# nubomedia/NUBOMEDIA-VCA

Measured on AMD Instinct MI355X. Metric: 1080p frames/sec/node (NuboFaceDetector); achieved HBM GB/s vs peak, higher is better.
Workload: dtype i32 rect sums / f32 products / f64 stage sums (u8 pixels)

## Files before the change

nubomedia-vca_amd/csrc/device_records.h:

```cpp
#pragma once
#include <stdint.h>
#include <stddef.h>

#if defined(__HIPCC__)
#define NVCA_HD __host__ __device__
#else
#define NVCA_HD
#endif

namespace nvca {

struct StageRec {
    int first, count; float thr;
    int flags;
    int thr_i;
    int vote_exp;
    int spec_run;
    int pad1;
};

struct ScaleRec {
    int    winw, winh;
    int    plane_off;
    int    pitch;
// ... 57 lines not shown
static constexpr int kTileLdsBudget = 52 * 1024;
static_assert(kTilesPerCu * kTileLdsBudget <= 160 * 1024 && kTilesPerCu * kTileThreads <= 32 * 64, "tile residency per CU");
static constexpr int kTileMaxCols = 256;
NVCA_HD inline int tile_pitch(int ncol) { return ncol | 1; }
NVCA_HD inline int tile_lds_fixed()
{
    return kTileSlots * 8 + 2 * kTileSlots * 2 + 4 * kTileWin + 128 + kTileSlots * 8;
}
NVCA_HD inline int tile_lds_bytes(int ncol, int nrow, int span_x, int span_y)
{
    return 4 * nrow * tile_pitch(ncol) + 2 * ((span_x + 3) & ~3) + 2 * ((span_y + 3) & ~3) + tile_lds_fixed();
}

static constexpr int kStripMaxWin = 512;
static constexpr int kIntegralBand = 16;

struct PreGeom {
    int sw, sh, sstride, cn;
    int w, h, gpitch;
    int spitch;
    int nbands;
    size_t src_slot, gray_slot, sum_slot, band_slot;
};
struct YuvPlanes {
    int fmt, cstride, vstride, pad;
    long long off_y, off_u, off_v;
};
struct ResizeView {
    int mode, xmax;
    const int *xofs; const short *ialpha; const int *yofs; const short *ibeta;
};
struct PyrLevelDev {
    int szw, szh, gpitch, plane_off;
    long long gray_off;
    ResizeView tab;
};
// ... 144 lines not shown
```

nubomedia-vca_amd/csrc/face_stream.cpp:

```cpp
#include "host_state.h"
#include "host_logic.h"
#include <algorithm>
#include <cstdio>
#include <new>

using namespace nvca;

struct nvca_face_stream {
    nvca_ctx *ctx;
    const nvca_cascade *cascade;
    nvca_face_params p;
    Faces faces;
    int num_frame = 0, num_iter = 0, frames_with_no_detection = 0, num_frames_to_process = 0;
    int pending_events = 0;
    nvca_pixel_layout input{};
    const nvca_pixel_layout *yuv() const { return input.format != NVCA_PIX_BGR ? &input : nullptr; }
};

namespace {
constexpr int kGOP = 4;
constexpr int kMaxNoDetection = 1;
constexpr int kNumFramesToProcess = 10;

struct FrameWork {
// ... 233 lines not shown
                hist_clean = nc;
            }
            ws.ln().hist_clean = 0;
            CascadeJob job; job.r0 = gbase + s0; job.n = nc; job.total = n;
            unsigned long long *z_hits = nullptr, *z_deep = nullptr;
            if (!lbp && (rc = cascade_counters(ctx, gp->det, job, &z_hits, &z_deep))) return rc;
            if (yuv) {
              TimedLaunch t(ctx, NVCA_K_GRAY);
              const bool wide = launch_gray_yuv(ctx->cs(), ws.res[ws.cur_res].srcptrs.as<const uint8_t *>() + gbase + s0, gp->g, yuv_planes(yuv), gp->view(),
                              ws.ln().gray.as<uint8_t>(), ws.ln().hist.as<unsigned>(), nc, frames_yuv_aligned16(frames, idx.data() + s0, nc, *yuv));
              if (ctx->sw.plan_debug) fprintf(stderr, "[nvca plan] %s gray of %d frame(s) %d x %d -> %d x %d: %s\n", yuv_is_422(yuv->format) ? "4:2:2" : "4:2:0", nc, f0.width, f0.height, cols, rows, gray_yuv_kernel_name(yuv->format, wide));
            } else
            { TimedLaunch t(ctx, NVCA_K_GRAY);
              launch_gray(ctx->cs(), ws.res[ws.cur_res].srcptrs.as<const uint8_t *>() + gbase + s0, gp->g, gp->view(),
                          ws.ln().gray.as<uint8_t>(), ws.ln().hist.as<unsigned>(), nc, frames_aligned4(frames, idx.data() + s0, nc)); }
            { TimedLaunch t(ctx, NVCA_K_LUT);
              launch_lut(ctx->cs(), ws.ln().hist.as<unsigned>(), cols * rows, ws.ln().lut.as<uint8_t>(), nc, 1, z_hits, z_deep); }
            job.counters_zeroed = !lbp;
            ws.ln().hist_clean = hist_clean;
            if (lbp) {
                const PyrSource src{ws.ln().gray.as<uint8_t>(), gp->g.gpitch, gp->g.gray_slot, ws.ln().lut.as<uint8_t>()};
                if (!scan->lv.empty()) { if ((rc = lbp_launch_set(ctx, scan, src, cols, rows, nc, job, gthr.data() + s0, tk.band_done))) return rc; }
                else { if ((rc = empty_job(ctx, job))) return rc; NVCA_HIP_CHECK(ctx, hipEventRecord(tk.band_done, ctx->cs())); }
            } else {
            run_integral(ctx, gp->g, ws.ln().lut.as<uint8_t>(), nc);
            if (streams[idx[0]]->cascade->c.has_tilted && (rc = run_tilted(ctx, gp->g, ws.ln().lut.as<uint8_t>(), nc))) return rc;
            if ((rc = cascade_enqueue(ctx, gp->det, gp->g.sum_slot, gp->g.spitch, job, gthr.data() + s0, true, tk.band_done))) return rc;
            }
            band_recorded = true;
            jobs.push_back(job);
        }
        gbase += batch;
    }
    if (!band_recorded) NVCA_HIP_CHECK(ctx, hipEventRecord(tk.band_done, ctx->cs()));
    if (!tk.done) NVCA_HIP_CHECK(ctx, hipEventCreateWithFlags(&tk.done, hipEventDisableTiming));
    NVCA_HIP_CHECK(ctx, hipEventRecord(tk.done, ctx->cs()));
    tk.pending = true;
    gates.armed = false;
    return NVCA_OK;
}
// ... 125 lines not shown
```

nubomedia-vca_amd/csrc/host_state.h:

```cpp
#pragma once
#include "context.h"
#include "plan.h"
#include "fb_search.h"
#include "host_math.h"
#include "pyr_levels.h"
#include "yuv_layout.h"

namespace nvca {

bool alloc_log();
void drain_timer_now(nvca_ctx *ctx);
void drain_timer(nvca_ctx *ctx);

struct ResultBufs {
    DevBuf hits, grp, gthr, staging, srcptrs;
    PinnedBuf h_hits, h_grp, h_gthr, h_srcptrs;
    DevBuf recs; PinnedBuf h_recs;
    std::vector<int> gthr_last;
    void release() { hits.release(); grp.release(); gthr.release(); staging.release(); srcptrs.release(); h_hits.release(); h_grp.release(); h_gthr.release(); h_srcptrs.release(); recs.release(); h_recs.release(); gthr_last.clear(); }
};
struct Lane {
    DevBuf gray, hist, lut, bandsum, bandsq, sum, sqsum, tilted, staging, aux, failbits, vnf, deep;
    int hist_clean = 0;
    void release_all()
    {
        gray.release(); hist.release(); lut.release(); bandsum.release(); bandsq.release(); sum.release();
        sqsum.release(); tilted.release(); staging.release(); aux.release();
        failbits.release(); vnf.release(); deep.release();
    }
};
struct Workspace {
    Lane lanes[kLanes];
    int *cur_lane = nullptr;
    Lane &ln() { return lanes[*cur_lane]; }
    ResultBufs res[3];
    int cur_res = 0;
    void release_all()
    {
        for (Lane &l : lanes) l.release_all();
        for (ResultBufs &r : res) r.release();
    }
// ... 41 lines not shown
    unsigned cap = 0;
    size_t first = 0;
    unsigned long long *d_hits = nullptr, *h_hits = nullptr;
    int *d_grp = nullptr, *h_grp = nullptr;
    LevelRec *d_recs = nullptr, *h_recs = nullptr;
};

struct TableBlob {
    std::vector<unsigned char> bytes;
    size_t add(const void *h, size_t n);
    int upload(nvca_ctx *ctx, DevBuf &blob);
};
void make_geom(PreGeom &g, int sw, int sh, int sstride, int cn, int w, int h);
int ensure_ws(nvca_ctx *ctx, const PreGeom &g, int batch);
int upload_tabs(nvca_ctx *ctx, std::vector<std::unique_ptr<GeomPlan>> &levels, DevBuf &blob);
void run_integral(nvca_ctx *ctx, const PreGeom &g, const uint8_t *lut, int batch, const uint8_t *gray = nullptr, int *sum = nullptr,
                  unsigned long long *sq = nullptr);
int run_tilted(nvca_ctx *ctx, const PreGeom &g, const uint8_t *lut, int batch, const uint8_t *gray = nullptr, int *tilted = nullptr);
int cascade_counters(nvca_ctx *ctx, DetectPlan &dp, const CascadeJob &job, unsigned long long **hits, unsigned long long **deep);
int cascade_enqueue(nvca_ctx *ctx, DetectPlan &dp, size_t sum_slot, int spitch, CascadeJob &job, const int *group_thr, bool want_group,
                    hipEvent_t early_done = nullptr );
int group_prepare(nvca_ctx *ctx, CascadeJob &job, const int *group_thr);
int cascade_fetch(nvca_ctx *ctx, CascadeJob &job);
int cascade_collect(nvca_ctx *ctx, DetectPlan &dp, const CascadeJob &job, std::vector<std::vector<nvca_rect>> &raw,
                    std::vector<char> *grouped, std::vector<std::vector<int>> *scale_of = nullptr,
                    std::vector<std::vector<LevelRec>> *recs = nullptr );
void group_all(std::vector<std::vector<nvca_rect>> &raw, int min_neighbors);
GeomPlan *find_plan(nvca_ctx *ctx, const std::string &key);
GeomPlan *store_plan(nvca_ctx *ctx, const std::string &key, std::unique_ptr<GeomPlan> gp);
int get_face_plan(nvca_ctx *ctx, const nvca_cascade *casc, int W, int H, int stride, int cn, int cols, int rows,
                  double sf, int minw, int minh, int maxw, int maxh, GeomPlan **out, const nvca_pixel_layout *yuv = nullptr);
int get_face_pre_plan(nvca_ctx *ctx, int W, int H, int stride, int cn, int cols, int rows, GeomPlan **out, const nvca_pixel_layout *yuv = nullptr);
// ... 98 lines not shown
```

nubomedia-vca_amd/csrc/kernels_equalize.hip:

```cpp
#include "launch.h"
#include "pre_device.h"

namespace nvca {

__global__ __launch_bounds__(256) void k_lut(unsigned *__restrict__ hist, int total, uint8_t *__restrict__ lut, int rezero,
                                             unsigned long long *__restrict__ zero_a, unsigned long long *__restrict__ zero_b)
{
    __shared__ unsigned wsum[4];
    __shared__ unsigned long long wmask[4];
    __shared__ unsigned hs[256];
    const int tid = threadIdx.x, lane = tid & 63, wave = tid >> 6, slot = blockIdx.x;
    const unsigned h = hist[slot * 256 + tid];
    hs[tid] = h;
    if (rezero) hist[slot * 256 + tid] = 0;
    if (slot == 0 && tid == 0) { if (zero_a) *zero_a = 0; if (zero_b) *zero_b = 0; }
    unsigned incl = h;
    for (int d = 1; d < 64; d <<= 1) { unsigned t = __shfl_up(incl, d); if (lane >= d) incl += t; }
    const unsigned long long m = __ballot(h != 0);
    if (lane == 63) wsum[wave] = incl;
    if (lane == 0) wmask[wave] = m;
    __syncthreads();
    for (int j = 0; j < wave; j++) incl += wsum[j];
    int first = 256;
    for (int j = 3; j >= 0; j--) if (wmask[j]) first = j * 64 + __ffsll((long long)wmask[j]) - 1;
    uint8_t out;
    if (first == 256) out = 0;
    else {
        const unsigned hf = hs[first];
        if (hf == (unsigned)total) out = (uint8_t)first;
        else if (tid <= first) out = 0;
        else {
            const float scale = 255.f / (float)(int)(total - (int)hf);
            const float v = (float)(int)(incl - hf) * scale;
            int iv = (int)rintf(v);
            out = (uint8_t)(iv < 0 ? 0 : (iv > 255 ? 255 : iv));
        }
    }
    lut[slot * 256 + tid] = out;
}

void launch_lut(hipStream_t st, unsigned *hist, int total, uint8_t *lut, int batch, int rezero, unsigned long long *zero_a,
                unsigned long long *zero_b)
{
    NVCA_LAUNCH(k_lut, dim3(batch), dim3(256), 0, st, hist, total, lut, rezero, zero_a, zero_b);
}

__global__ __launch_bounds__(256) void k_hist(const uint8_t *__restrict__ gray, int w, int h, int pitch,
                                              unsigned *__restrict__ hist)
{
    __shared__ unsigned lh[4][256];
    const int tid = threadIdx.x, wave = tid >> 6;
    for (int i = tid; i < 1024; i += 256) (&lh[0][0])[i] = 0;
    __syncthreads();
// ... 53 lines not shown
```

nubomedia-vca_amd/csrc/kernels_integral.hip:

```cpp
#include "launch.h"

namespace nvca {

__global__ __launch_bounds__(256) void k_colsum(const uint8_t *__restrict__ gray, const uint8_t *__restrict__ lut,
                                                int lut_stride, PreGeom g, unsigned *__restrict__ bandsum,
                                                unsigned *__restrict__ bandsq)
{
    __shared__ uint8_t sl[256];
    const int tid = threadIdx.x, band = blockIdx.y, slot = blockIdx.z;
    sl[tid] = lut ? lut[(size_t)slot * lut_stride + tid] : (uint8_t)tid;
    __syncthreads();
    const int x4 = (blockIdx.x * 256 + tid) * 4;
    const int bpitch = (int)(g.band_slot / g.nbands);
    if (x4 >= bpitch) return;
    const int y0 = band * kIntegralBand, y1 = min(g.h, y0 + kIntegralBand);
    unsigned s[4] = {0, 0, 0, 0}, q[4] = {0, 0, 0, 0};
    if (x4 < g.w) {
        const uint8_t *base = gray + (size_t)slot * g.gray_slot + x4;
        for (int y = y0; y < y1; y++) {
            const unsigned px = *(const unsigned *)(base + (size_t)y * g.gpitch);
#pragma unroll
            for (int k = 0; k < 4; k++) {
                const unsigned v = (x4 + k < g.w) ? sl[(px >> (8 * k)) & 255] : 0u;
                s[k] += v; q[k] += v * v;
            }
        }
    }
    const size_t o = (size_t)slot * g.band_slot + (size_t)band * bpitch + x4;
    *(uint4 *)(bandsum + o) = make_uint4(s[0], s[1], s[2], s[3]);
    *(uint4 *)(bandsq + o) = make_uint4(q[0], q[1], q[2], q[3]);
}
void launch_colsum(hipStream_t st, const uint8_t *gray, const uint8_t *lut, int lut_stride, const PreGeom &g,
                   unsigned *bandsum, unsigned *bandsq, int batch)
{
    const int bpitch = (int)(g.band_slot / g.nbands);
    dim3 grid((bpitch / 4 + 255) / 256, g.nbands, batch);
    NVCA_LAUNCH(k_colsum, grid, dim3(256), 0, st, gray, lut, lut_stride, g, bandsum, bandsq);
}

__global__ __launch_bounds__(256) void k_bandscan(PreGeom g, unsigned *__restrict__ bandsum, unsigned *__restrict__ bandsq)
{
    const int bpitch = (int)(g.band_slot / g.nbands);
    const int x = blockIdx.x * 256 + threadIdx.x, slot = blockIdx.y;
    if (x >= bpitch) return;
    unsigned rs = 0, rq = 0;
    size_t o = (size_t)slot * g.band_slot + x;
    for (int b0 = 0; b0 < g.nbands; b0 += 16) {
        unsigned ts[16], tq[16];
#pragma unroll
        for (int k = 0; k < 16; k++) {
            const bool in = b0 + k < g.nbands;
            ts[k] = in ? bandsum[o + (size_t)k * bpitch] : 0u; tq[k] = in ? bandsq[o + (size_t)k * bpitch] : 0u;
        }
#pragma unroll
        for (int k = 0; k < 16; k++)
            if (b0 + k < g.nbands) {
                bandsum[o + (size_t)k * bpitch] = rs; bandsq[o + (size_t)k * bpitch] = rq;
                rs += ts[k]; rq += tq[k];
            }
        o += (size_t)16 * bpitch;
    }
}
void launch_bandscan(hipStream_t st, const PreGeom &g, unsigned *bandsum, unsigned *bandsq, int batch)
{
    const int bpitch = (int)(g.band_slot / g.nbands);
    NVCA_LAUNCH(k_bandscan, dim3((bpitch + 255) / 256, batch), dim3(256), 0, st, g, bandsum, bandsq);
}

__device__ __forceinline__ unsigned wave_incl_scan_u32(unsigned v, int lane)
{
    unsigned x = v;
    x += (unsigned)__builtin_amdgcn_update_dpp(0, (int)v, 0x111, 0xf, 0xf, true);
    x += (unsigned)__builtin_amdgcn_update_dpp(0, (int)v, 0x112, 0xf, 0xf, true);
    x += (unsigned)__builtin_amdgcn_update_dpp(0, (int)v, 0x113, 0xf, 0xf, true);
    x += (unsigned)__builtin_amdgcn_update_dpp(0, (int)x, 0x114, 0xf, 0xe, true);
    x += (unsigned)__builtin_amdgcn_update_dpp(0, (int)x, 0x118, 0xf, 0xc, true);
    const unsigned t0 = (unsigned)__builtin_amdgcn_readlane((int)x, 15), t1 = (unsigned)__builtin_amdgcn_readlane((int)x, 31),
                   t2 = (unsigned)__builtin_amdgcn_readlane((int)x, 47);
    const int row = lane >> 4;
    return x + (row >= 1 ? t0 : 0u) + (row >= 2 ? t1 : 0u) + (row >= 3 ? t2 : 0u);
}

static constexpr int kIntThreads = 512;
static constexpr int kIntWaves = kIntThreads / 64;

__global__ __launch_bounds__(kIntThreads) void k_integral(const uint8_t *__restrict__ gray, const uint8_t *__restrict__ lut,
                                                          int lut_stride, PreGeom g, const unsigned *__restrict__ bandsum,
                                                          const unsigned *__restrict__ bandsq, int *__restrict__ sum,
                                                          unsigned *__restrict__ sq32)
{
    __shared__ uint8_t sl[256];
    __shared__ unsigned wrow_s[kIntegralBand][kIntWaves], wrow_q[kIntegralBand][kIntWaves];
    __shared__ unsigned wb_s[kIntWaves];
    __shared__ unsigned long long wb_q[kIntWaves];
    __shared__ unsigned carry_s[kIntegralBand], carry_q[kIntegralBand];
    __shared__ unsigned cbase_s;
    __shared__ unsigned long long cbase_q;
    const int tid = threadIdx.x, lane = tid & 63, wave = tid >> 6;
    const int band = blockIdx.x, slot = blockIdx.y;
    if (tid < 256) sl[tid] = lut ? lut[(size_t)slot * lut_stride + tid] : (uint8_t)tid;
    if (tid < kIntegralBand) { carry_s[tid] = 0; carry_q[tid] = 0; }
    if (tid == 0) { cbase_s = 0; cbase_q = 0; }
    __syncthreads();
    const int y0 = band * kIntegralBand, y1 = min(g.h, y0 + kIntegralBand);
    const int bpitch = (int)(g.band_slot / g.nbands);
    const uint8_t *gbase = gray + (size_t)slot * g.gray_slot;
    int *sbase = sum + (size_t)slot * g.sum_slot;
    unsigned *lbase = sq32 + (size_t)slot * 2 * g.sum_slot;
    uint8_t *hbase = (uint8_t *)(lbase + g.sum_slot);
    const unsigned *bs = bandsum + (size_t)slot * g.band_slot + (size_t)band * bpitch;
    const unsigned *bq = bandsq + (size_t)slot * g.band_slot + (size_t)band * bpitch;
    const int nchunks = (g.w + 1 + 2047) / 2048;

    for (int c = 0; c < nchunks; c++) {
        const int X0 = c * 2048 + tid * 4;
        const bool in_pitch = X0 < g.spitch;
        unsigned ps[4]; unsigned long long pq[4];
        {
            uint4 a = make_uint4(0, 0, 0, 0), e = make_uint4(0, 0, 0, 0);
            if (X0 + 4 <= bpitch) { a = *(const uint4 *)(bs + X0); e = *(const uint4 *)(bq + X0); }
            const unsigned vs[4] = {a.x, a.y, a.z, a.w}, vq[4] = {e.x, e.y, e.z, e.w};
            unsigned rs = 0; unsigned long long rq = 0;
#pragma unroll
            for (int k = 0; k < 4; k++) {
                const bool ok = X0 + k < g.w;
                rs += ok ? vs[k] : 0u; rq += ok ? vq[k] : 0u;
                ps[k] = rs; pq[k] = rq;
            }
        }
        const unsigned ts = ps[3]; const unsigned long long tq = pq[3];
        unsigned is = wave_incl_scan_u32(ts + (tid == 0 ? cbase_s : 0u), lane);
        unsigned long long iq = tq + (tid == 0 ? cbase_q : 0ull);
        for (int d = 1; d < 64; d <<= 1) { const unsigned long long b = __shfl_up(iq, d); if (lane >= d) iq += b; }
        if (lane == 63) { wb_s[wave] = is; wb_q[wave] = iq; }
        __syncthreads();
        for (int j = 0; j < wave; j++) { is += wb_s[j]; iq += wb_q[j]; }
// ... 53 lines not shown
                *(unsigned *)(hbase + o) = (unsigned)(acc_q[0] >> 32) | ((unsigned)(acc_q[1] >> 32) << 8) | ((unsigned)(acc_q[2] >> 32) << 16) |
                                           ((unsigned)(acc_q[3] >> 32) << 24);
            }
            }
        }
        __syncthreads();
        if (tid < kIntegralBand) {
            unsigned ts_ = 0, tq_ = 0;
            for (int j = 0; j < kIntWaves; j++) { ts_ += wrow_s[tid][j]; tq_ += wrow_q[tid][j]; }
            carry_s[tid] += ts_; carry_q[tid] += tq_;
        }
        __syncthreads();
    }
}
void launch_integral(hipStream_t st, const uint8_t *gray, const uint8_t *lut, int lut_stride, const PreGeom &g,
                     const unsigned *bandsum, const unsigned *bandsq, int *sum, unsigned long long *sqsum,
                     int batch)
{
    NVCA_LAUNCH(k_integral, dim3(g.nbands, batch), dim3(kIntThreads), 0, st, gray, lut, lut_stride, g, bandsum,
                       bandsq, sum, (unsigned *)sqsum);
}

static constexpr int kSmallIntWords = 16 * 1024 - 256;
__device__ __forceinline__ void small_integral(const uint8_t *__restrict__ g, int gpitch, const uint8_t *__restrict__ lut, int w, int h,
                                               int *__restrict__ s, unsigned *__restrict__ lo, uint8_t *__restrict__ hi, int P, unsigned *sm)
{
    const int tid = threadIdx.x, lane = tid & 63, wave = tid >> 6, nthreads = blockDim.x, nwaves = nthreads >> 6;
    const int pitch = w | 1;
    for (int X = tid; X <= w; X += nthreads) { s[X] = 0; lo[X] = 0; hi[X] = 0; }
    for (int pass = 0; pass < 2; pass++) {
        for (int y = wave; y < h; y += nwaves) {
            const uint8_t *row = g + (size_t)y * gpitch;
            unsigned carry = 0;
            for (int x0 = 0; x0 < w; x0 += 64) {
                const int x = x0 + lane;
// ... 148 lines not shown
```

nubomedia-vca_amd/csrc/launch.h:

```cpp
#pragma once
#include <hip/hip_runtime.h>
#include <hip/hip_ext.h>
#include "device_records.h"
#include "trk_layout.h"
#include "pixel_rules.h"

namespace nvca {

bool launch_events(hipEvent_t *a, hipEvent_t *b);
void note_launch(const char *kernel);
hipError_t take_launch_error(const char **kernel);
#define NVCA_LAUNCH(kern, grid, block, shmem, st, ...)                                                            \
    do {                                                                                                          \
        hipEvent_t ea__, eb__;                                                                                    \
        if (nvca::launch_events(&ea__, &eb__)) hipExtLaunchKernelGGL(kern, grid, block, shmem, st, ea__, eb__, 0, __VA_ARGS__); \
        else hipLaunchKernelGGL(kern, grid, block, shmem, st, __VA_ARGS__);                                       \
        nvca::note_launch(#kern);                                                                                 \
    } while (0)

void launch_gray(hipStream_t st, const uint8_t *const *d_src, const PreGeom &g, const ResizeView &t,
                 uint8_t *gray, unsigned *hist, int batch, bool aligned4);
bool launch_gray_yuv(hipStream_t st, const uint8_t *const *d_src, const PreGeom &g, const YuvPlanes &p, const ResizeView &t,
                     uint8_t *gray, unsigned *hist, int batch, bool aligned16);
const char *gray_yuv_kernel_name(int fmt, bool wide);
// ... 7 lines not shown
void launch_resize1(hipStream_t st, const uint8_t *src, int sw, int sh, int sstride, const ResizeView &t,
                    uint8_t *dst, int dw, int dh, int dstride, unsigned *hist, int batch = 1, size_t src_slot = 0, size_t dst_slot = 0,
                    const uint8_t *luts = nullptr );
void launch_resize3(hipStream_t st, const uint8_t *src, int sw, int sh, int sstride, const ResizeView &t,
                    uint8_t *dst, int dw, int dh, int dstride);
void launch_flip_h(hipStream_t st, const uint8_t *src, int w, int h, int spitch, uint8_t *dst, int dpitch, int batch = 1, size_t src_slot = 0,
                   size_t dst_slot = 0);
void launch_hist(hipStream_t st, const uint8_t *gray, int w, int h, int pitch, unsigned *hist);
void launch_lut(hipStream_t st, unsigned *hist, int total, uint8_t *lut, int batch, int rezero = 0,
                unsigned long long *zero_a = nullptr, unsigned long long *zero_b = nullptr);
void launch_apply_lut(hipStream_t st, const uint8_t *src, int w, int h, int spitch, const uint8_t *lut,
                      uint8_t *dst, int dpitch, int batch = 1, size_t src_slot = 0, size_t dst_slot = 0);
void launch_work_resize(hipStream_t st, bool bgr, const uint8_t *const *d_srcs, const int *d_lut_idx, const uint8_t *d_luts, int sh, int sstride,
                        const ResizeView &t, uint8_t *dst, int dw, int dh, int dstride, size_t dst_slot, unsigned *hist, int batch, const YuvPlanes *yuv = nullptr);
void launch_colsum(hipStream_t st, const uint8_t *gray, const uint8_t *lut, int lut_stride, const PreGeom &g,
                   unsigned *bandsum, unsigned *bandsq, int batch);
void launch_bandscan(hipStream_t st, const PreGeom &g, unsigned *bandsum, unsigned *bandsq, int batch);
void launch_integral(hipStream_t st, const uint8_t *gray, const uint8_t *lut, int lut_stride, const PreGeom &g,
                     const unsigned *bandsum, const unsigned *bandsq, int *sum, unsigned long long *sqsum,
                     int batch);

bool small_integral_fits(const PreGeom &g);
void launch_small_integral(hipStream_t st, const uint8_t *gray, const uint8_t *lut, int lut_stride, const PreGeom &g, int *sum,
                           unsigned long long *sqsum, int batch);

struct TrkLaunch {
    const TrkSlot *slots; int batch, w, h;
    int fmt;
    bool wide;
    int *labels; CompAcc *acc;
    int *out; int cap;
    uint8_t *flags; int *roots; int roots_cap; int *tiles; int tick;
    int order;
    int rows, rows_uf;
};
// ... 55 lines not shown
```

nubomedia-vca_amd/csrc/plans.cpp:

```cpp
#include "host_state.h"
#include "host_logic.h"
#include <cstdio>
#include <cstring>
#include <algorithm>

using namespace nvca;

namespace nvca {

static RowCopy make_rowcopy(const ResizeTab &t)
{
    RowCopy rc;
    if (t.mode != 1 || t.dh <= 0) return rc;
    std::vector<int> rows;
    auto clampr = [&](int r) { return r >= 0 ? (r < t.sh ? r : t.sh - 1) : 0; };
    for (int dy = 0; dy < t.dh; dy++) { rows.push_back(clampr(t.yofs[dy])); rows.push_back(clampr(t.yofs[dy] + 1)); }
    std::sort(rows.begin(), rows.end());
    rows.erase(std::unique(rows.begin(), rows.end()), rows.end());
    if (rows.size() * 2 > (size_t)t.sh) return rc;
    std::vector<std::pair<int, int>> runs;
    for (int r : rows) { if (!runs.empty() && runs.back().first + runs.back().second == r) runs.back().second++; else runs.push_back({r, 1}); }
    const int period = runs.size() > 1 ? runs[1].first - runs[0].first : t.sh;
    for (size_t i = 0; i < runs.size(); i++)
        if (runs[i].second != runs[0].second || runs[i].first != runs[0].first + (int)i * period) return rc;
// ... 46 lines not shown
    for (auto &it : items) it.d->release();
    int rc;
    if ((rc = blob.upload(ctx, d_blob))) return rc;
    for (auto &it : items) { it.d->p = it.n ? (unsigned char *)d_blob.p + it.off : nullptr; it.d->bytes = 0; }
    return NVCA_OK;
}

void make_geom(PreGeom &g, int sw, int sh, int sstride, int cn, int w, int h)
{
    memset(&g, 0, sizeof(g));
    g.sw = sw; g.sh = sh; g.sstride = sstride; g.cn = cn;
    g.w = w; g.h = h;
    g.gpitch = (int)round_up(w, 64);
    g.spitch = (int)round_up(w + 1, 8);
    g.nbands = (h + kIntegralBand - 1) / kIntegralBand;
    g.gray_slot = round_up((size_t)g.gpitch * h, 256);
    g.sum_slot = round_up((size_t)g.spitch * (h + 1), 64);
    g.band_slot = (size_t)g.nbands * round_up(w, 8);
}

int ensure_ws(nvca_ctx *ctx, const PreGeom &g, int batch)
{
    Workspace &ws = *ctx->ws;
    int e = 0;
    e |= ws.ln().gray.ensure(g.gray_slot * batch + 64);
    { void *old = ws.ln().hist.p; e |= ws.ln().hist.ensure((size_t)batch * 256 * sizeof(unsigned)); if (ws.ln().hist.p != old) ws.ln().hist_clean = 0; }
    e |= ws.ln().lut.ensure((size_t)batch * 256);
    e |= ws.ln().bandsum.ensure(g.band_slot * batch * sizeof(unsigned));
    e |= ws.ln().bandsq.ensure(g.band_slot * batch * sizeof(unsigned));
    e |= ws.ln().sum.ensure((g.sum_slot * batch + 4 * (size_t)g.spitch) * sizeof(int));
    e |= ws.ln().sqsum.ensure(g.sum_slot * batch * sizeof(unsigned long long));
    e |= ws.res[ws.cur_res].srcptrs.ensure((size_t)batch * sizeof(void *));
    e |= ws.res[ws.cur_res].h_srcptrs.ensure((size_t)batch * sizeof(void *));
    if (e) { ctx->set_error("device/pinned allocation failed for the workspace"); return NVCA_ERR_NOMEM; }
    return NVCA_OK;
}

static int upload_tab(nvca_ctx *ctx, GeomPlan &gp)
{
    const ResizeTab &t = gp.tab;
    if (t.mode != 1) return NVCA_OK;
    if (gp.d_xofs.ensure(t.xofs.size() * 4) || gp.d_yofs.ensure(t.yofs.size() * 4) ||
        gp.d_ialpha.ensure(t.ialpha.size() * 2) || gp.d_ibeta.ensure(t.ibeta.size() * 2)) {
        ctx->set_error("hipMalloc failed for resize tables"); return NVCA_ERR_NOMEM;
// ... 14 lines not shown
    std::vector<unsigned char> h(total);
    if (blob.ensure(total)) { ctx->set_error("hipMalloc failed for resize tables"); return NVCA_ERR_NOMEM; }
    size_t off = 0;
    auto put = [&](DevBuf &d, const void *src, size_t n) { memcpy(h.data() + off, src, n); d.release(); d.p = (unsigned char *)blob.p + off; d.bytes = 0; off += al(n); };
    for (auto &gp : levels) {
        const ResizeTab &t = gp->tab;
        if (t.mode != 1) continue;
        put(gp->d_xofs, t.xofs.data(), t.xofs.size() * 4); put(gp->d_yofs, t.yofs.data(), t.yofs.size() * 4);
        put(gp->d_ialpha, t.ialpha.data(), t.ialpha.size() * 2); put(gp->d_ibeta, t.ibeta.data(), t.ibeta.size() * 2);
    }
    NVCA_HIP_CHECK(ctx, hipMemcpy(blob.p, h.data(), total, hipMemcpyHostToDevice));
    return NVCA_OK;
}


void run_integral(nvca_ctx *ctx, const PreGeom &g, const uint8_t *lut, int batch, const uint8_t *gray, int *sum,
                  unsigned long long *sq)
{
    Workspace &ws = *ctx->ws;
    if (!gray) gray = ws.ln().gray.as<uint8_t>();
    if (!sum) sum = ws.ln().sum.as<int>();
    if (!sq) sq = ws.ln().sqsum.as<unsigned long long>();
    if (batch <= 64 && small_integral_fits(g)) {
        TimedLaunch t(ctx, NVCA_K_INTEGRAL);
        launch_small_integral(ctx->cs(), gray, lut, 256, g, sum, sq, batch);
        return;
    }
    { TimedLaunch t(ctx, NVCA_K_COLSUM);
      launch_colsum(ctx->cs(), gray, lut, 256, g, ws.ln().bandsum.as<unsigned>(), ws.ln().bandsq.as<unsigned>(), batch); }
    { TimedLaunch t(ctx, NVCA_K_BANDSCAN);
      launch_bandscan(ctx->cs(), g, ws.ln().bandsum.as<unsigned>(), ws.ln().bandsq.as<unsigned>(), batch); }
    { TimedLaunch t(ctx, NVCA_K_INTEGRAL);
      launch_integral(ctx->cs(), gray, lut, 256, g, ws.ln().bandsum.as<unsigned>(), ws.ln().bandsq.as<unsigned>(), sum, sq, batch); }
}

int run_tilted(nvca_ctx *ctx, const PreGeom &g, const uint8_t *lut, int batch, const uint8_t *gray, int *tilted)
{
    Workspace &ws = *ctx->ws;
    if (g.w + 1 > 8 * 1024 || (size_t)2 * (g.w + g.h + 2) * sizeof(int) > 64 * 1024) { ctx->set_error("image too large for the tilted integral"); return NVCA_ERR_ARG; }
    if (!tilted) {
        if (ws.ln().tilted.ensure((g.sum_slot * batch + 4 * (size_t)g.spitch) * sizeof(int))) { ctx->set_error("device allocation failed (tilted integral)"); return NVCA_ERR_NOMEM; }
        tilted = ws.ln().tilted.as<int>();
    }
    if (!gray) gray = ws.ln().gray.as<uint8_t>();
    TimedLaunch t(ctx, NVCA_K_INTEGRAL);
    launch_tilted(ctx->cs(), gray, lut, 256, g, tilted, batch);
    return NVCA_OK;
}
// ... 305 lines not shown
```

nubomedia-vca_amd/csrc/pre_device.h:

```cpp
#pragma once
#include "launch.h"

#if defined(__HIPCC__)
namespace nvca {

static constexpr int kGrayRows = 8;

__device__ __forceinline__ void hist_flush(unsigned (*lh)[256], unsigned *hist, int tid)
{
    __syncthreads();
    unsigned v = lh[0][tid] + lh[1][tid] + lh[2][tid] + lh[3][tid];
    if (v) atomicAdd(&hist[tid], v);
}

}
#endif
```

Baseline: 21130.

## Fuse histogram-equalize LUT into colsum and scan super-bands instead of all bands

Removes the separate LUT launch on the multi-launch integral path: colsum now builds the equalization LUT from the histogram itself and writes it out once, and bandscan takes over re-zeroing the histogram and counters. Colsum is restructured so each thread loads 16 pixels per row with wide loads across four bands per block and emits band prefixes within a super-band of four bands. The serial band scan then runs only over super-band totals, and the integral kernel adds the super-band prefix back in. This cuts one launch and shortens the serial scan, at the cost of redundant per-block LUT computation and more shared memory and register use in colsum.

```diff
diff --git a/nubomedia-vca_amd/csrc/device_records.h b/nubomedia-vca_amd/csrc/device_records.h
--- a/nubomedia-vca_amd/csrc/device_records.h
+++ b/nubomedia-vca_amd/csrc/device_records.h
@@ -95,12 +95,13 @@
 
 static constexpr int kStripMaxWin = 512;
 static constexpr int kIntegralBand = 16;
+static constexpr int kSuperBands = 4;
 
 struct PreGeom {
     int sw, sh, sstride, cn;
     int w, h, gpitch;
     int spitch;
-    int nbands;
+    int nbands, nsuper;
     size_t src_slot, gray_slot, sum_slot, band_slot;
 };
 struct YuvPlanes {
diff --git a/nubomedia-vca_amd/csrc/face_stream.cpp b/nubomedia-vca_amd/csrc/face_stream.cpp
--- a/nubomedia-vca_amd/csrc/face_stream.cpp
+++ b/nubomedia-vca_amd/csrc/face_stream.cpp
@@ -271,16 +271,20 @@
             { TimedLaunch t(ctx, NVCA_K_GRAY);
               launch_gray(ctx->cs(), ws.res[ws.cur_res].srcptrs.as<const uint8_t *>() + gbase + s0, gp->g, gp->view(),
                           ws.ln().gray.as<uint8_t>(), ws.ln().hist.as<unsigned>(), nc, frames_aligned4(frames, idx.data() + s0, nc)); }
-            { TimedLaunch t(ctx, NVCA_K_LUT);
-              launch_lut(ctx->cs(), ws.ln().hist.as<unsigned>(), cols * rows, ws.ln().lut.as<uint8_t>(), nc, 1, z_hits, z_deep); }
+            const bool chain_lut = !lbp && !integral_in_one_launch(gp->g, nc);
+            const ChainEqualize eq{ws.ln().hist.as<unsigned>(), cols * rows, ws.ln().lut.as<uint8_t>(), z_hits, z_deep};
+            if (!chain_lut) {
+              TimedLaunch t(ctx, NVCA_K_LUT);
+              launch_lut(ctx->cs(), ws.ln().hist.as<unsigned>(), cols * rows, ws.ln().lut.as<uint8_t>(), nc, 1, z_hits, z_deep);
+              ws.ln().hist_clean = hist_clean; }
             job.counters_zeroed = !lbp;
-            ws.ln().hist_clean = hist_clean;
             if (lbp) {
                 const PyrSource src{ws.ln().gray.as<uint8_t>(), gp->g.gpitch, gp->g.gray_slot, ws.ln().lut.as<uint8_t>()};
                 if (!scan->lv.empty()) { if ((rc = lbp_launch_set(ctx, scan, src, cols, rows, nc, job, gthr.data() + s0, tk.band_done))) return rc; }
                 else { if ((rc = empty_job(ctx, job))) return rc; NVCA_HIP_CHECK(ctx, hipEventRecord(tk.band_done, ctx->cs())); }
             } else {
-            run_integral(ctx, gp->g, ws.ln().lut.as<uint8_t>(), nc);
+            run_integral(ctx, gp->g, ws.ln().lut.as<uint8_t>(), nc, nullptr, nullptr, nullptr, chain_lut ? &eq : nullptr);
+            if (chain_lut) ws.ln().hist_clean = hist_clean;
             if (streams[idx[0]]->cascade->c.has_tilted && (rc = run_tilted(ctx, gp->g, ws.ln().lut.as<uint8_t>(), nc))) return rc;
             if ((rc = cascade_enqueue(ctx, gp->det, gp->g.sum_slot, gp->g.spitch, job, gthr.data() + s0, true, tk.band_done))) return rc;
             }
diff --git a/nubomedia-vca_amd/csrc/host_state.h b/nubomedia-vca_amd/csrc/host_state.h
--- a/nubomedia-vca_amd/csrc/host_state.h
+++ b/nubomedia-vca_amd/csrc/host_state.h
@@ -20,11 +20,11 @@
     void release() { hits.release(); grp.release(); gthr.release(); staging.release(); srcptrs.release(); h_hits.release(); h_grp.release(); h_gthr.release(); h_srcptrs.release(); recs.release(); h_recs.release(); gthr_last.clear(); }
 };
 struct Lane {
-    DevBuf gray, hist, lut, bandsum, bandsq, sum, sqsum, tilted, staging, aux, failbits, vnf, deep;
+    DevBuf gray, hist, lut, bandsum, bandsq, supersum, supersq, sum, sqsum, tilted, staging, aux, failbits, vnf, deep;
     int hist_clean = 0;
     void release_all()
     {
-        gray.release(); hist.release(); lut.release(); bandsum.release(); bandsq.release(); sum.release();
+        gray.release(); hist.release(); lut.release(); bandsum.release(); bandsq.release(); supersum.release(); supersq.release(); sum.release();
         sqsum.release(); tilted.release(); staging.release(); aux.release();
         failbits.release(); vnf.release(); deep.release();
     }
@@ -96,8 +96,13 @@
 void make_geom(PreGeom &g, int sw, int sh, int sstride, int cn, int w, int h);
 int ensure_ws(nvca_ctx *ctx, const PreGeom &g, int batch);
 int upload_tabs(nvca_ctx *ctx, std::vector<std::unique_ptr<GeomPlan>> &levels, DevBuf &blob);
+struct ChainEqualize {
+    unsigned *hist; int total; uint8_t *lut;
+    unsigned long long *zero_a, *zero_b;
+};
+bool integral_in_one_launch(const PreGeom &g, int batch);
 void run_integral(nvca_ctx *ctx, const PreGeom &g, const uint8_t *lut, int batch, const uint8_t *gray = nullptr, int *sum = nullptr,
-                  unsigned long long *sq = nullptr);
+                  unsigned long long *sq = nullptr, const ChainEqualize *eq = nullptr );
 int run_tilted(nvca_ctx *ctx, const PreGeom &g, const uint8_t *lut, int batch, const uint8_t *gray = nullptr, int *tilted = nullptr);
 int cascade_counters(nvca_ctx *ctx, DetectPlan &dp, const CascadeJob &job, unsigned long long **hits, unsigned long long **deep);
 int cascade_enqueue(nvca_ctx *ctx, DetectPlan &dp, size_t sum_slot, int spitch, CascadeJob &job, const int *group_thr, bool want_group,
diff --git a/nubomedia-vca_amd/csrc/kernels_equalize.hip b/nubomedia-vca_amd/csrc/kernels_equalize.hip
--- a/nubomedia-vca_amd/csrc/kernels_equalize.hip
+++ b/nubomedia-vca_amd/csrc/kernels_equalize.hip
@@ -6,37 +6,12 @@
 __global__ __launch_bounds__(256) void k_lut(unsigned *__restrict__ hist, int total, uint8_t *__restrict__ lut, int rezero,
                                              unsigned long long *__restrict__ zero_a, unsigned long long *__restrict__ zero_b)
 {
-    __shared__ unsigned wsum[4];
-    __shared__ unsigned long long wmask[4];
-    __shared__ unsigned hs[256];
-    const int tid = threadIdx.x, lane = tid & 63, wave = tid >> 6, slot = blockIdx.x;
+    __shared__ LutScratch sc;
+    const int tid = threadIdx.x, slot = blockIdx.x;
     const unsigned h = hist[slot * 256 + tid];
-    hs[tid] = h;
     if (rezero) hist[slot * 256 + tid] = 0;
     if (slot == 0 && tid == 0) { if (zero_a) *zero_a = 0; if (zero_b) *zero_b = 0; }
-    unsigned incl = h;
-    for (int d = 1; d < 64; d <<= 1) { unsigned t = __shfl_up(incl, d); if (lane >= d) incl += t; }
-    const unsigned long long m = __ballot(h != 0);
-    if (lane == 63) wsum[wave] = incl;
-    if (lane == 0) wmask[wave] = m;
-    __syncthreads();
-    for (int j = 0; j < wave; j++) incl += wsum[j];
-    int first = 256;
-    for (int j = 3; j >= 0; j--) if (wmask[j]) first = j * 64 + __ffsll((long long)wmask[j]) - 1;
-    uint8_t out;
-    if (first == 256) out = 0;
-    else {
-        const unsigned hf = hs[first];
-        if (hf == (unsigned)total) out = (uint8_t)first;
-        else if (tid <= first) out = 0;
-        else {
-            const float scale = 255.f / (float)(int)(total - (int)hf);
-            const float v = (float)(int)(incl - hf) * scale;
-            int iv = (int)rintf(v);
-            out = (uint8_t)(iv < 0 ? 0 : (iv > 255 ? 255 : iv));
-        }
-    }
-    lut[slot * 256 + tid] = out;
+    lut[slot * 256 + tid] = equalize_lut_entry(h, total, tid, sc);
 }
 
 void launch_lut(hipStream_t st, unsigned *hist, int total, uint8_t *lut, int batch, int rezero, unsigned long long *zero_a,
diff --git a/nubomedia-vca_amd/csrc/kernels_integral.hip b/nubomedia-vca_amd/csrc/kernels_integral.hip
--- a/nubomedia-vca_amd/csrc/kernels_integral.hip
+++ b/nubomedia-vca_amd/csrc/kernels_integral.hip
@@ -1,70 +1,152 @@
 #include "launch.h"
+#include "pre_device.h"
 
 namespace nvca {
 
-__global__ __launch_bounds__(256) void k_colsum(const uint8_t *__restrict__ gray, const uint8_t *__restrict__ lut,
-                                                int lut_stride, PreGeom g, unsigned *__restrict__ bandsum,
-                                                unsigned *__restrict__ bandsq)
+static constexpr int kColsumWaves = 4;
+static constexpr int kColsumCols = 64 * 16;
+template <bool kWide>
+__device__ __forceinline__ void colsum_load(uint4 (&px)[kIntegralBand], const uint8_t *__restrict__ p, int pitch, int x0, int w, int nr)
+{
+#pragma unroll
+    for (int r = 0; r < kIntegralBand; r++) {
+        px[r] = make_uint4(0, 0, 0, 0);
+        if (x0 < w && r < nr) {
+            const uint8_t *row = p + (size_t)r * pitch;
+            if (kWide) px[r] = *(const uint4 *)row;
+            else {
+                px[r].x = *(const unsigned *)row;
+                if (x0 + 4 < w) px[r].y = *(const unsigned *)(row + 4);
+                if (x0 + 8 < w) px[r].z = *(const unsigned *)(row + 8);
+                if (x0 + 12 < w) px[r].w = *(const unsigned *)(row + 12);
+            }
+        }
+    }
+}
+template <bool kWide>
+__global__ __launch_bounds__(kColsumWaves * 64) void k_colsum(const uint8_t *__restrict__ gray, const uint8_t *__restrict__ lut, int lut_stride,
+                                                              PreGeom g, unsigned *__restrict__ bandsum, unsigned *__restrict__ bandsq,
+                                                              unsigned *__restrict__ supersum, unsigned *__restrict__ supersq,
+                                                              const unsigned *__restrict__ hist, int total, uint8_t *__restrict__ lut_out)
 {
     __shared__ uint8_t sl[256];
-    const int tid = threadIdx.x, band = blockIdx.y, slot = blockIdx.z;
-    sl[tid] = lut ? lut[(size_t)slot * lut_stride + tid] : (uint8_t)tid;
+    __shared__ LutScratch sc;
+    __shared__ __attribute__((aligned(16))) unsigned sm_s[kSuperBands][kColsumCols], sm_q[kSuperBands][kColsumCols];
+    const int tid = threadIdx.x, lane = tid & 63, wave = __builtin_amdgcn_readfirstlane(tid >> 6);
+    const int sb = blockIdx.y, slot = blockIdx.z;
+    const int bpitch = (int)(g.band_slot / g.nbands);
+    const int xb = blockIdx.x * kColsumCols, x0 = xb + lane * 16;
+    const uint8_t *base = gray + (size_t)slot * g.gray_slot + x0;
+    uint4 px[kIntegralBand];
+    int bi = wave;
+    int y0 = (sb * kSuperBands + bi) * kIntegralBand, nr = min(kIntegralBand, g.h - y0);
+    if (bi < kSuperBands) colsum_load<kWide>(px, base + (size_t)y0 * g.gpitch, g.gpitch, x0, g.w, nr);
+    if (hist) {
+        const uint8_t e = equalize_lut_entry(hist[slot * 256 + tid], total, tid, sc);
+        sl[tid] = e;
+        if (blockIdx.x == 0 && sb == 0) lut_out[(size_t)slot * lut_stride + tid] = e;
+    } else sl[tid] = lut ? lut[(size_t)slot * lut_stride + tid] : (uint8_t)tid;
     __syncthreads();
-    const int x4 = (blockIdx.x * 256 + tid) * 4;
+    while (bi < kSuperBands) {
+        unsigned s[16], q[16];
+#pragma unroll
+        for (int k = 0; k < 16; k++) { s[k] = 0; q[k] = 0; }
+#pragma unroll
+        for (int r = 0; r < kIntegralBand; r++)
+            if (r < nr) {
+                const unsigned wd[4] = {px[r].x, px[r].y, px[r].z, px[r].w};
+#pragma unroll
+                for (int k = 0; k < 16; k++) {
+                    const unsigned v = sl[(wd[k >> 2] >> (8 * (k & 3))) & 255];
+                    s[k] += v; q[k] += v * v;
+                }
+            }
+#pragma unroll
+        for (int k = 0; k < 16; k += 4) {
+            *(uint4 *)&sm_s[bi][lane * 16 + k] = make_uint4(s[k], s[k + 1], s[k + 2], s[k + 3]);
+            *(uint4 *)&sm_q[bi][lane * 16 + k] = make_uint4(q[k], q[k + 1], q[k + 2], q[k + 3]);
+        }
+        bi += kColsumWaves;
+        if (bi < kSuperBands) {
+            y0 = (sb * kSuperBands + bi) * kIntegralBand; nr = min(kIntegralBand, g.h - y0);
+            colsum_load<kWide>(px, base + (size_t)y0 * g.gpitch, g.gpitch, x0, g.w, nr);
+        }
+    }
+    __syncthreads();
+    for (bi = wave; bi < kSuperBands; bi += kColsumWaves) {
+        const int band = sb * kSuperBands + bi;
+        const bool last = bi == kSuperBands - 1;
+        if (band >= g.nbands && !last) continue;
+#pragma unroll
+        for (int i = 0; i < kColsumCols / 256; i++) {
+            const int c = (i * 64 + lane) * 4;
+            if (xb + c + 4 > bpitch) continue;
+            uint4 as = make_uint4(0, 0, 0, 0), aq = make_uint4(0, 0, 0, 0);
+            for (int j = 0; j < bi; j++) {
+                const uint4 ts = *(const uint4 *)&sm_s[j][c], tq = *(const uint4 *)&sm_q[j][c];
+                as.x += ts.x; as.y += ts.y; as.z += ts.z; as.w += ts.w;
+                aq.x += tq.x; aq.y += tq.y; aq.z += tq.z; aq.w += tq.w;
+            }
+            if (band < g.nbands) {
+                const size_t o = (size_t)slot * g.band_slot + (size_t)band * bpitch + xb + c;
+                *(uint4 *)(bandsum + o) = as; *(uint4 *)(bandsq + o) = aq;
+            }
+            if (last) {
+                const uint4 ts = *(const uint4 *)&sm_s[bi][c], tq = *(const uint4 *)&sm_q[bi][c];
+                as.x += ts.x; as.y += ts.y; as.z += ts.z; as.w += ts.w;
+                aq.x += tq.x; aq.y += tq.y; aq.z += tq.z; aq.w += tq.w;
+                const size_t o = ((size_t)slot * g.nsuper + sb) * bpitch + xb + c;
+                *(uint4 *)(supersum + o) = as; *(uint4 *)(supersq + o) = aq;
+            }
+        }
+    }
+}
+void launch_colsum(hipStream_t st, const uint8_t *gray, const uint8_t *lut, int lut_stride, const PreGeom &g,
+                   unsigned *bandsum, unsigned *bandsq, unsigned *supersum, unsigned *supersq, int batch,
+                   const unsigned *hist, int total, uint8_t *lut_out)
+{
     const int bpitch = (int)(g.band_slot / g.nbands);
-    if (x4 >= bpitch) return;
-    const int y0 = band * kIntegralBand, y1 = min(g.h, y0 + kIntegralBand);
-    unsigned s[4] = {0, 0, 0, 0}, q[4] = {0, 0, 0, 0};
-    if (x4 < g.w) {
-        const uint8_t *base = gray + (size_t)slot * g.gray_slot + x4;
-        for (int y = y0; y < y1; y++) {
-            const unsigned px = *(const unsigned *)(base + (size_t)y * g.gpitch);
-#pragma unroll
-            for (int k = 0; k < 4; k++) {
-                const unsigned v = (x4 + k < g.w) ? sl[(px >> (8 * k)) & 255] : 0u;
-                s[k] += v; q[k] += v * v;
-            }
-        }
-    }
-    const size_t o = (size_t)slot * g.band_slot + (size_t)band * bpitch + x4;
-    *(uint4 *)(bandsum + o) = make_uint4(s[0], s[1], s[2], s[3]);
-    *(uint4 *)(bandsq + o) = make_uint4(q[0], q[1], q[2], q[3]);
-}
-void launch_colsum(hipStream_t st, const uint8_t *gray, const uint8_t *lut, int lut_stride, const PreGeom &g,
-                   unsigned *bandsum, unsigned *bandsq, int batch)
-{
-    const int bpitch = (int)(g.band_slot / g.nbands);
-    dim3 grid((bpitch / 4 + 255) / 256, g.nbands, batch);
-    NVCA_LAUNCH(k_colsum, grid, dim3(256), 0, st, gray, lut, lut_stride, g, bandsum, bandsq);
-}
-
-__global__ __launch_bounds__(256) void k_bandscan(PreGeom g, unsigned *__restrict__ bandsum, unsigned *__restrict__ bandsq)
+    dim3 grid((bpitch + kColsumCols - 1) / kColsumCols, g.nsuper, batch);
+    if (!(((uintptr_t)gray | (uintptr_t)g.gpitch | (uintptr_t)g.gray_slot) & 15))
+        NVCA_LAUNCH(k_colsum<true>, grid, dim3(kColsumWaves * 64), 0, st, gray, lut, lut_stride, g, bandsum, bandsq, supersum, supersq, hist, total, lut_out);
+    else
+        NVCA_LAUNCH(k_colsum<false>, grid, dim3(kColsumWaves * 64), 0, st, gray, lut, lut_stride, g, bandsum, bandsq, supersum, supersq, hist, total, lut_out);
+}
+
+__global__ __launch_bounds__(256) void k_bandscan(PreGeom g, unsigned *__restrict__ supersum, unsigned *__restrict__ supersq,
+                                                  unsigned *__restrict__ hist, unsigned long long *__restrict__ zero_a,
+                                                  unsigned long long *__restrict__ zero_b)
 {
     const int bpitch = (int)(g.band_slot / g.nbands);
     const int x = blockIdx.x * 256 + threadIdx.x, slot = blockIdx.y;
+    if (blockIdx.x == 0) {
+        if (hist) hist[slot * 256 + threadIdx.x] = 0;
+        if (slot == 0 && threadIdx.x == 0) { if (zero_a) *zero_a = 0; if (zero_b) *zero_b = 0; }
+    }
     if (x >= bpitch) return;
     unsigned rs = 0, rq = 0;
-    size_t o = (size_t)slot * g.band_slot + x;
-    for (int b0 = 0; b0 < g.nbands; b0 += 16) {
+    size_t o = (size_t)slot * g.nsuper * bpitch + x;
+    for (int b0 = 0; b0 < g.nsuper; b0 += 16) {
         unsigned ts[16], tq[16];
 #pragma unroll
         for (int k = 0; k < 16; k++) {
-            const bool in = b0 + k < g.nbands;
-            ts[k] = in ? bandsum[o + (size_t)k * bpitch] : 0u; tq[k] = in ? bandsq[o + (size_t)k * bpitch] : 0u;
+            const bool in = b0 + k < g.nsuper;
+            ts[k] = in ? supersum[o + (size_t)k * bpitch] : 0u; tq[k] = in ? supersq[o + (size_t)k * bpitch] : 0u;
         }
 #pragma unroll
         for (int k = 0; k < 16; k++)
-            if (b0 + k < g.nbands) {
-                bandsum[o + (size_t)k * bpitch] = rs; bandsq[o + (size_t)k * bpitch] = rq;
+            if (b0 + k < g.nsuper) {
+                supersum[o + (size_t)k * bpitch] = rs; supersq[o + (size_t)k * bpitch] = rq;
                 rs += ts[k]; rq += tq[k];
             }
         o += (size_t)16 * bpitch;
     }
 }
-void launch_bandscan(hipStream_t st, const PreGeom &g, unsigned *bandsum, unsigned *bandsq, int batch)
+void launch_bandscan(hipStream_t st, const PreGeom &g, unsigned *supersum, unsigned *supersq, int batch, unsigned *hist,
+                     unsigned long long *zero_a, unsigned long long *zero_b)
 {
     const int bpitch = (int)(g.band_slot / g.nbands);
-    NVCA_LAUNCH(k_bandscan, dim3((bpitch + 255) / 256, batch), dim3(256), 0, st, g, bandsum, bandsq);
+    NVCA_LAUNCH(k_bandscan, dim3((bpitch + 255) / 256, batch), dim3(256), 0, st, g, supersum, supersq, hist, zero_a, zero_b);
 }
 
 __device__ __forceinline__ unsigned wave_incl_scan_u32(unsigned v, int lane)
@@ -86,7 +168,8 @@
 
 __global__ __launch_bounds__(kIntThreads) void k_integral(const uint8_t *__restrict__ gray, const uint8_t *__restrict__ lut,
                                                           int lut_stride, PreGeom g, const unsigned *__restrict__ bandsum,
-                                                          const unsigned *__restrict__ bandsq, int *__restrict__ sum,
+                                                          const unsigned *__restrict__ bandsq, const unsigned *__restrict__ supersum,
+                                                          const unsigned *__restrict__ supersq, int *__restrict__ sum,
                                                           unsigned *__restrict__ sq32)
 {
     __shared__ uint8_t sl[256];
@@ -110,6 +193,8 @@
     uint8_t *hbase = (uint8_t *)(lbase + g.sum_slot);
     const unsigned *bs = bandsum + (size_t)slot * g.band_slot + (size_t)band * bpitch;
     const unsigned *bq = bandsq + (size_t)slot * g.band_slot + (size_t)band * bpitch;
+    const unsigned *ss = supersum + ((size_t)slot * g.nsuper + band / kSuperBands) * bpitch;
+    const unsigned *sq = supersq + ((size_t)slot * g.nsuper + band / kSuperBands) * bpitch;
     const int nchunks = (g.w + 1 + 2047) / 2048;
 
     for (int c = 0; c < nchunks; c++) {
@@ -118,8 +203,9 @@
         unsigned ps[4]; unsigned long long pq[4];
         {
             uint4 a = make_uint4(0, 0, 0, 0), e = make_uint4(0, 0, 0, 0);
-            if (X0 + 4 <= bpitch) { a = *(const uint4 *)(bs + X0); e = *(const uint4 *)(bq + X0); }
-            const unsigned vs[4] = {a.x, a.y, a.z, a.w}, vq[4] = {e.x, e.y, e.z, e.w};
+            uint4 ta = a, te = e;
+            if (X0 + 4 <= bpitch) { a = *(const uint4 *)(bs + X0); e = *(const uint4 *)(bq + X0); ta = *(const uint4 *)(ss + X0); te = *(const uint4 *)(sq + X0); }
+            const unsigned vs[4] = {a.x + ta.x, a.y + ta.y, a.z + ta.z, a.w + ta.w}, vq[4] = {e.x + te.x, e.y + te.y, e.z + te.z, e.w + te.w};
             unsigned rs = 0; unsigned long long rq = 0;
 #pragma unroll
             for (int k = 0; k < 4; k++) {
@@ -203,11 +289,11 @@
     }
 }
 void launch_integral(hipStream_t st, const uint8_t *gray, const uint8_t *lut, int lut_stride, const PreGeom &g,
-                     const unsigned *bandsum, const unsigned *bandsq, int *sum, unsigned long long *sqsum,
-                     int batch)
+                     const unsigned *bandsum, const unsigned *bandsq, const unsigned *supersum, const unsigned *supersq,
+                     int *sum, unsigned long long *sqsum, int batch)
 {
     NVCA_LAUNCH(k_integral, dim3(g.nbands, batch), dim3(kIntThreads), 0, st, gray, lut, lut_stride, g, bandsum,
-                       bandsq, sum, (unsigned *)sqsum);
+                       bandsq, supersum, supersq, sum, (unsigned *)sqsum);
 }
 
 static constexpr int kSmallIntWords = 16 * 1024 - 256;
diff --git a/nubomedia-vca_amd/csrc/launch.h b/nubomedia-vca_amd/csrc/launch.h
--- a/nubomedia-vca_amd/csrc/launch.h
+++ b/nubomedia-vca_amd/csrc/launch.h
@@ -45,11 +45,13 @@
 void launch_work_resize(hipStream_t st, bool bgr, const uint8_t *const *d_srcs, const int *d_lut_idx, const uint8_t *d_luts, int sh, int sstride,
                         const ResizeView &t, uint8_t *dst, int dw, int dh, int dstride, size_t dst_slot, unsigned *hist, int batch, const YuvPlanes *yuv = nullptr);
 void launch_colsum(hipStream_t st, const uint8_t *gray, const uint8_t *lut, int lut_stride, const PreGeom &g,
-                   unsigned *bandsum, unsigned *bandsq, int batch);
-void launch_bandscan(hipStream_t st, const PreGeom &g, unsigned *bandsum, unsigned *bandsq, int batch);
+                   unsigned *bandsum, unsigned *bandsq, unsigned *supersum, unsigned *supersq, int batch,
+                   const unsigned *hist = nullptr, int total = 0, uint8_t *lut_out = nullptr);
+void launch_bandscan(hipStream_t st, const PreGeom &g, unsigned *supersum, unsigned *supersq, int batch, unsigned *hist = nullptr,
+                     unsigned long long *zero_a = nullptr, unsigned long long *zero_b = nullptr);
 void launch_integral(hipStream_t st, const uint8_t *gray, const uint8_t *lut, int lut_stride, const PreGeom &g,
-                     const unsigned *bandsum, const unsigned *bandsq, int *sum, unsigned long long *sqsum,
-                     int batch);
+                     const unsigned *bandsum, const unsigned *bandsq, const unsigned *supersum, const unsigned *supersq,
+                     int *sum, unsigned long long *sqsum, int batch);
 
 bool small_integral_fits(const PreGeom &g);
 void launch_small_integral(hipStream_t st, const uint8_t *gray, const uint8_t *lut, int lut_stride, const PreGeom &g, int *sum,
diff --git a/nubomedia-vca_amd/csrc/plans.cpp b/nubomedia-vca_amd/csrc/plans.cpp
--- a/nubomedia-vca_amd/csrc/plans.cpp
+++ b/nubomedia-vca_amd/csrc/plans.cpp
@@ -84,6 +84,7 @@
     g.gpitch = (int)round_up(w, 64);
     g.spitch = (int)round_up(w + 1, 8);
     g.nbands = (h + kIntegralBand - 1) / kIntegralBand;
+    g.nsuper = (g.nbands + kSuperBands - 1) / kSuperBands;
     g.gray_slot = round_up((size_t)g.gpitch * h, 256);
     g.sum_slot = round_up((size_t)g.spitch * (h + 1), 64);
     g.band_slot = (size_t)g.nbands * round_up(w, 8);
@@ -98,6 +99,8 @@
     e |= ws.ln().lut.ensure((size_t)batch * 256);
     e |= ws.ln().bandsum.ensure(g.band_slot * batch * sizeof(unsigned));
     e |= ws.ln().bandsq.ensure(g.band_slot * batch * sizeof(unsigned));
+    e |= ws.ln().supersum.ensure(g.band_slot / g.nbands * g.nsuper * batch * sizeof(unsigned));
+    e |= ws.ln().supersq.ensure(g.band_slot / g.nbands * g.nsuper * batch * sizeof(unsigned));
     e |= ws.ln().sum.ensure((g.sum_slot * batch + 4 * (size_t)g.spitch) * sizeof(int));
     e |= ws.ln().sqsum.ensure(g.sum_slot * batch * sizeof(unsigned long long));
     e |= ws.res[ws.cur_res].srcptrs.ensure((size_t)batch * sizeof(void *));
@@ -142,24 +145,30 @@
 }
 
 
+bool integral_in_one_launch(const PreGeom &g, int batch) { return batch <= 64 && small_integral_fits(g); }
+
 void run_integral(nvca_ctx *ctx, const PreGeom &g, const uint8_t *lut, int batch, const uint8_t *gray, int *sum,
-                  unsigned long long *sq)
+                  unsigned long long *sq, const ChainEqualize *eq)
 {
     Workspace &ws = *ctx->ws;
     if (!gray) gray = ws.ln().gray.as<uint8_t>();
     if (!sum) sum = ws.ln().sum.as<int>();
     if (!sq) sq = ws.ln().sqsum.as<unsigned long long>();
-    if (batch <= 64 && small_integral_fits(g)) {
+    if (integral_in_one_launch(g, batch)) {
         TimedLaunch t(ctx, NVCA_K_INTEGRAL);
         launch_small_integral(ctx->cs(), gray, lut, 256, g, sum, sq, batch);
         return;
     }
+    unsigned *bs = ws.ln().bandsum.as<unsigned>(), *bq = ws.ln().bandsq.as<unsigned>();
+    unsigned *ss = ws.ln().supersum.as<unsigned>(), *ssq = ws.ln().supersq.as<unsigned>();
     { TimedLaunch t(ctx, NVCA_K_COLSUM);
-      launch_colsum(ctx->cs(), gray, lut, 256, g, ws.ln().bandsum.as<unsigned>(), ws.ln().bandsq.as<unsigned>(), batch); }
+      if (eq) launch_colsum(ctx->cs(), gray, nullptr, 256, g, bs, bq, ss, ssq, batch, eq->hist, eq->total, eq->lut);
+      else launch_colsum(ctx->cs(), gray, lut, 256, g, bs, bq, ss, ssq, batch); }
     { TimedLaunch t(ctx, NVCA_K_BANDSCAN);
-      launch_bandscan(ctx->cs(), g, ws.ln().bandsum.as<unsigned>(), ws.ln().bandsq.as<unsigned>(), batch); }
+      if (eq) launch_bandscan(ctx->cs(), g, ss, ssq, batch, eq->hist, eq->zero_a, eq->zero_b);
+      else launch_bandscan(ctx->cs(), g, ss, ssq, batch); }
     { TimedLaunch t(ctx, NVCA_K_INTEGRAL);
-      launch_integral(ctx->cs(), gray, lut, 256, g, ws.ln().bandsum.as<unsigned>(), ws.ln().bandsq.as<unsigned>(), sum, sq, batch); }
+      launch_integral(ctx->cs(), gray, eq ? eq->lut : lut, 256, g, bs, bq, ss, ssq, sum, sq, batch); }
 }
 
 int run_tilted(nvca_ctx *ctx, const PreGeom &g, const uint8_t *lut, int batch, const uint8_t *gray, int *tilted)
diff --git a/nubomedia-vca_amd/csrc/pre_device.h b/nubomedia-vca_amd/csrc/pre_device.h
--- a/nubomedia-vca_amd/csrc/pre_device.h
+++ b/nubomedia-vca_amd/csrc/pre_device.h
@@ -13,5 +13,33 @@
     if (v) atomicAdd(&hist[tid], v);
 }
 
+struct LutScratch {
+    unsigned hs[256];
+    unsigned wsum[4];
+    unsigned long long wmask[4];
+};
+__device__ __forceinline__ uint8_t equalize_lut_entry(unsigned h, int total, int tid, LutScratch &sc)
+{
+    const int lane = tid & 63, wave = tid >> 6;
+    sc.hs[tid] = h;
+    unsigned incl = h;
+    for (int d = 1; d < 64; d <<= 1) { unsigned t = __shfl_up(incl, d); if (lane >= d) incl += t; }
+    const unsigned long long m = __ballot(h != 0);
+    if (lane == 63) sc.wsum[wave] = incl;
+    if (lane == 0) sc.wmask[wave] = m;
+    __syncthreads();
+    for (int j = 0; j < wave; j++) incl += sc.wsum[j];
+    int first = 256;
+    for (int j = 3; j >= 0; j--) if (sc.wmask[j]) first = j * 64 + __ffsll((long long)sc.wmask[j]) - 1;
+    if (first == 256) return 0;
+    const unsigned hf = sc.hs[first];
+    if (hf == (unsigned)total) return (uint8_t)first;
+    if (tid <= first) return 0;
+    const float scale = 255.f / (float)(int)(total - (int)hf);
+    const float v = (float)(int)(incl - hf) * scale;
+    const int iv = (int)rintf(v);
+    return (uint8_t)(iv < 0 ? 0 : (iv > 255 ? 255 : iv));
+}
+
 }
 #endif
```

Result: no change. 21310, median of 6 (+0.8%).
